# shamspias/fennec

Hardware: AMD Instinct MI355X
Metric: megapixels/sec: 4K SSIMFast+GaussianBlur (higher is better)
Workload: dtype u8 (blur: exact int32 sums of 24-bit fixed-point weights on the i8 matrix pipe; fp64 SSIM)

## Files before the change

### fennec_amd/csrc/blur_mfma.hip

```cpp
#include <hip/hip_ext.h>

#include "blur_launch.hpp"
#include "devutil.hpp"

#include <algorithm>
#include <cmath>
#include <type_traits>
#include <vector>

namespace fnx {

typedef int v4i __attribute__((ext_vector_type(4)));

constexpr int MF_P = 48;
constexpr int MF_WT = 64 * MF_P + 256;
constexpr int MF_SP = 352;
constexpr int MF_OP = 272;

__host__ __device__ constexpr int mf_skew(int grp) { return 80 * grp; }
static_assert(64 * MF_P + mf_skew(3) <= MF_WT, "the ring's last group ends inside the wave's ring");

struct MfmaArgs {
    const uint8_t *src;
    const uint8_t *const *srcs;
    uint8_t *dst;
    uint8_t *const *dsts;
    int sstride, dstride, w, h;
    int tiles_x, tiles, seg;
    int radius;
    const uint32_t *tab;
    int seed_h, seed_v, thr;
    const int32_t *bx, *by;
    const uint32_t *coltab, *rowtab;
    unsigned long long *slabs;
    int nbx, nby;
    int dbg;
    int narrow;
};

__device__ __forceinline__ int mf_comb3(int hi, int mid, int lo)
{
    int t = hi * 256 + mid;
    asm volatile("" : "+v"(t));
    return t * 256 + lo;
}

__device__ __forceinline__ const double *mf_scalar_ptr(const double *p)
{
    const unsigned long long v = reinterpret_cast<unsigned long long>(p);
    const unsigned lo = __builtin_amdgcn_readfirstlane(static_cast<unsigned>(v)), hi = __builtin_amdgcn_readfirstlane(static_cast<unsigned>(v >> 32));
    return reinterpret_cast<const double *>((static_cast<unsigned long long>(hi) << 32) | lo);
}
typedef __attribute__((address_space(1))) uint8_t mf_g_u8;
template <typename T> __device__ __forceinline__ T *mf_sgpr_ptr(T *p)
{
    unsigned long long v = reinterpret_cast<unsigned long long>(p);
    asm volatile("" : "+s"(v));
    return reinterpret_cast<T *>(v);
}
__device__ __forceinline__ void mf_lane_off(uint32_t &o) { asm volatile("" : "+v"(o)); }
typedef int mf_s16i __attribute__((ext_vector_type(16)));
__device__ __forceinline__ uint32_t mf_exact_u(const double *wd, const uint8_t *base, int step, int ring0, int mask)
{
    mf_s16i w0, w1;
    asm volatile("s_load_dwordx16 %0, %2, 0x0\n\ts_load_dwordx16 %1, %2, 0x40\n\ts_waitcnt lgkmcnt(0)" : "=&s"(w0), "=&s"(w1) : "s"(mf_scalar_ptr(wd)) : "memory");
    uint32_t v[13];
#pragma unroll
    for (int t = 0; t < 13; t++) v[t] = base[((ring0 + t) & mask) * step];
    double acc = 0;
#pragma unroll
    for (int t = 0; t < 13; t++) {
        const int lo = t < 8 ? w0[2 * (t & 7)] : w1[2 * (t & 7)], hi = t < 8 ? w0[2 * (t & 7) + 1] : w1[2 * (t & 7) + 1];
        acc = acc + u8_to_f64(v[t] ^ 0x80u) * __hiloint2double(hi, lo);
    }
    return clampF_dev(acc);
}

__device__ __forceinline__ void mf_box_add4(uint32_t *tbl, const u32x4 ro, uint32_t coln, const v4i cb, bool live)
{
    if (!live) return;
#pragma unroll
    for (int k = 0; k < 4; k++)
        __hip_atomic_fetch_add(reinterpret_cast<uint32_t *>(reinterpret_cast<char *>(tbl) + ro[k] + coln), static_cast<uint32_t>(cb[k]),
                               __ATOMIC_RELAXED, __HIP_MEMORY_SCOPE_WORKGROUP);
}

template <bool SCORE, bool GUARD>
__global__ __launch_bounds__(256, GUARD ? 3 : 1) void blur_mfma_kernel(MfmaArgs a)
{
    constexpr int P = MF_P, WT = MF_WT, SP = MF_SP, OP = MF_OP;
    __shared__ __attribute__((aligned(16))) uint8_t s_t[4 * WT];
    __shared__ __attribute__((aligned(16))) uint8_t s_stage[2 * 16 * SP];
    __shared__ __attribute__((aligned(16))) uint8_t s_out[2 * 16 * OP];
    __shared__ __attribute__((aligned(16))) uint32_t s_rowh[SCORE ? MF_SEG_SCORE + 32 : 4];
    __shared__ __attribute__((aligned(16))) uint32_t s_rowv[SCORE ? MF_SEG_SCORE + 16 : 4];
    extern __shared__ __attribute__((aligned(16))) uint32_t s_box[];

    const int tile = xcd_tile(blockIdx.x, a.tiles);
    if (tile < 0) return;
    const int z = blockIdx.y;
    const uint8_t *src = a.srcs ? a.srcs[z] : a.src;
    uint8_t *dst = a.dsts ? a.dsts[z] : a.dst;
    const int ty = tile / a.tiles_x, tx = tile - ty * a.tiles_x;
    const int x0 = tx * 64, y0 = ty * a.seg;
    const int tid = threadIdx.x, wave = tid >> 6, lane = tid & 63;
    const int r = lane & 15, g = lane >> 4;
    const int NJ = min(a.seg, ((a.h - y0 + 15) >> 4) << 4) >> 4;
    const int NI = NJ + 1;
    const bool xedge = x0 - 6 < 0 || x0 + 70 > a.w;

    const v4i *tbh = reinterpret_cast<const v4i *>(a.tab);
    const long *tbv = reinterpret_cast<const long *>(a.tab + 3 * 64 * 4);
    const v4i bh2 = tbh[lane], bh1 = tbh[64 + lane], bh0 = tbh[128 + lane];
    const long bv2 = tbv[lane], bv1 = tbv[64 + lane], bv0 = tbv[128 + lane];
    const bool alane = (r & 3) == 3;
    const int seed_hl = alane ? (1 << 23) + 128 : a.seed_h;
    const v4i sh = {seed_hl, seed_hl, seed_hl, seed_hl}, sv = {a.seed_v, a.seed_v, a.seed_v, a.seed_v};
    const v4i zero = {0, 0, 0, 0};
    const uint32_t sel01 = alane ? 0x0c0c0400u : 0x0c0c0703u, sel23 = alane ? 0x04000c0cu : 0x07030c0cu;

    uint8_t *tw = s_t + wave * WT;
    const int id1 = min(256 + tid, 16 * 19 - 1);
    const int srow0 = tid / 19, sch0 = tid - 19 * srow0, srow1 = id1 / 19, sch1 = id1 - 19 * srow1;
    const bool two = tid < 48;
    const int st_w0 = srow0 * SP + 16 * sch0, st_w1 = srow1 * SP + 16 * sch1;
    const int st_r = r * SP + 64 * wave + 16 * g;
    uint8_t *t_w = tw + r * P + 4 * g;
    const int m4 = r >> 2, mi = r & 3;
    const uint8_t *t_r = tw + (16 * m4 + 4 * mi) * P + mf_skew(m4) + 8 * g;
    const uint8_t *t_ro = tw + (16 * m4 + 4 * mi) * P + mf_skew(m4) + ((8 * g + 16) & 31);
    const uint8_t *t_ae = tw + (16 * g + 3) * P + mf_skew(g) + r + 6;
    const uint8_t *t_ao = tw + (16 * g + 3) * P + mf_skew(g) + ((r + 22) & 31);
    const int o_w = r * OP + 64 * wave + 16 * g;
    const int orow = tid >> 4, och = tid & 15;
    const int o_r = orow * OP + 16 * och;
    const int xo = x0 + 4 * och;

    v4i bbox = {0, 0, 0, 0}, sbox = {0, 0, 0, 0};
    uint32_t coln = 0;
    bool live = false;
    const int slabn = SCORE ? (a.nbx + 1) * (a.nby + 1) : 0;
    uint32_t *tbl_s = s_box, *tbl_b = s_box + 4 * slabn;
    auto score_setup = [&]() {
        const uint32_t cw = a.coltab[256 * tx + tid];
        const int nrow = (2 * a.seg + 16) >> 2;
        const int nrh = (a.seg + 16) >> 2;
        const u32x4 rw = reinterpret_cast<const u32x4 *>(a.rowtab)[static_cast<size_t>(ty) * nrow + min(tid, nrow - 1)];
        if (!(a.dbg & 4)) for (int e = tid; e < 2 * slabn; e += 256) reinterpret_cast<u32x4 *>(s_box)[e] = (u32x4){0u, 0u, 0u, 0u};
        if (tid < nrh) reinterpret_cast<u32x4 *>(s_rowh)[tid] = rw;
        else if (tid < nrow) reinterpret_cast<u32x4 *>(s_rowv)[tid - nrh] = rw;
        coln = cw & 0xfffffu;
        live = cw >> 31;
        const int seed = static_cast<int>((cw >> 20) & 31u) << 7;
        sbox = (v4i){seed, seed, seed, seed};
        const uint32_t sh = ((cw >> 29) & 3u) << 3;
#pragma unroll
        for (int e = 0; e < 4; e++) bbox[e] = static_cast<int>(((cw >> (25 + e)) & 1u) << sh);
    };

    const double *wd = reinterpret_cast<const double *>(a.tab + 3 * 64 * 4 + 3 * 64 * 2);

    auto stage_write = [&](const u32x4 (&d)[2], int buf) {
        uint8_t *sb = s_stage + buf * 16 * SP;
        *reinterpret_cast<u32x4 *>(sb + st_w0) = d[0] ^ 0x80808080u;
        if (two) *reinterpret_cast<u32x4 *>(sb + st_w1) = d[1] ^ 0x80808080u;
    };
    auto hset = [&](int s, int buf, int slot) {
        const uint8_t *sbuf = s_stage + buf * 16 * SP;
        const uint8_t *sb = sbuf + st_r;
        if constexpr (!GUARD && !SCORE) {
#pragma unroll
            for (int hf = 0; hf < 2; hf++) {
                v4i c2[2], c1[2], c0[2];
#pragma unroll
                for (int q2 = 0; q2 < 2; q2++) {
                    const v4i A = *reinterpret_cast<const v4i *>(sb + 16 * (2 * hf + q2));
                    c2[q2] = __builtin_amdgcn_mfma_i32_16x16x64_i8(A, bh2, zero, 0, 0, 0);
                    c1[q2] = __builtin_amdgcn_mfma_i32_16x16x64_i8(A, bh1, zero, 0, 0, 0);
                    c0[q2] = __builtin_amdgcn_mfma_i32_16x16x64_i8(A, bh0, sh, 0, 0, 0);
                }
#pragma unroll
// ... 125 lines not shown
            if (__builtin_amdgcn_ballot_w64(mm < static_cast<uint32_t>(a.thr))) {
                uint32_t fl = 0;
#pragma unroll
                for (int q = 0; q < 3; q++)
#pragma unroll
                    for (int i = 0; i < 4; i++) fl |= ((static_cast<uint32_t>(u[q][i]) & 0x00ffffffu) < static_cast<uint32_t>(a.thr) ? 1u : 0u) << (4 * q + i);
                unsigned long long todo = __builtin_amdgcn_ballot_w64(fl != 0);
                while (todo) {
                    const int L = __builtin_ctzll(todo);
                    todo &= todo - 1;
                    uint32_t flL = __builtin_amdgcn_readlane(fl, L);
                    const int rL = L & 15, gL = L >> 4;
                    while (flL) {
                        const int b = __builtin_ctz(flL), q = b >> 2, i = b & 3;
                        flL &= flL - 1;
                        const uint32_t e = mf_exact_u(wd, tw + (16 * gL + 4 * i + q) * P + mf_skew(gL), 1, (ODD ? 16 : 0) + rL, 31);
                        if (lane == L) op[4 * i + q] = static_cast<uint8_t>(e);
                    }
                }
                if constexpr (SCORE) o = *reinterpret_cast<const u32x4 *>(op);
            }
        }
        if constexpr (SCORE) {
            const u32x4 os = o ^ 0x80808080u;
            const v4i A = {(int)os[0], (int)os[1], (int)os[2], (int)os[3]};
            const v4i cb = __builtin_amdgcn_mfma_i32_16x16x64_i8(A, bbox, sbox, 0, 0, 0);
            const u32x4 ro = *reinterpret_cast<const u32x4 *>(s_rowv + 16 * j + 4 * g);
            if (!(a.dbg & 1)) mf_box_add4(tbl_b, ro, coln, cb, live);
        }
    };

    auto march = [&](auto formt) {
        constexpr int FORM = decltype(formt)::value;
        constexpr bool XEDGE = FORM == 2, INNER = FORM == 0;
        const uint8_t *in_base = INNER ? src + static_cast<ptrdiff_t>(y0 - 6) * a.sstride + 4 * static_cast<ptrdiff_t>(x0 - 6) : src;
        uint8_t *out_base = INNER ? dst + static_cast<ptrdiff_t>(y0) * a.dstride + 4 * static_cast<ptrdiff_t>(x0) : dst;
        const uint32_t ss = static_cast<uint32_t>(a.sstride), ds = static_cast<uint32_t>(a.dstride);
        const uint32_t in_set = 16u * ss, out_set = 16u * ds;
        uint32_t in_l0 = static_cast<uint32_t>(srow0) * ss + 16u * sch0, in_l1 = static_cast<uint32_t>(srow1) * ss + 16u * sch1;
        uint32_t out_l = static_cast<uint32_t>(orow) * ds + 16u * och;
        auto hload = [&](int i, u32x4 (&d)[2]) {
            const int ys = y0 - 6 + 16 * i;
            if constexpr (INNER) {
                const mf_g_u8 *sb = (const mf_g_u8 *)mf_sgpr_ptr(in_base + static_cast<uint32_t>(i) * in_set);
                mf_lane_off(in_l0);
                mf_lane_off(in_l1);
                d[0] = *(g_u32x4 *)(sb + in_l0);
                d[1] = *(g_u32x4 *)(sb + in_l1);
            } else if constexpr (!XEDGE) {
                const uint8_t *sb = src + 4 * static_cast<ptrdiff_t>(x0 - 6);
                const int ya = clampi(ys + srow0, 0, a.h - 1), yb = clampi(ys + srow1, 0, a.h - 1);
                d[0] = *(g_u32x4 *)(sb + static_cast<ptrdiff_t>(ya) * a.sstride + 16 * sch0);
                d[1] = *(g_u32x4 *)(sb + static_cast<ptrdiff_t>(yb) * a.sstride + 16 * sch1);
            } else {
    #pragma unroll
                for (int k = 0; k < 2; k++) {
                    if (k == 1 && !two) break;
                    const int y = clampi(ys + (k ? srow1 : srow0), 0, a.h - 1);
                    const uint8_t *rowp = src + static_cast<size_t>(y) * a.sstride;
                    const int xc = x0 - 6 + 4 * (k ? sch1 : sch0);
    #pragma unroll
                    for (int e = 0; e < 4; e++) d[k][e] = ld_px(rowp, clampi(xc + e, 0, a.w - 1));
                }
            }
        };
        auto out_store = [&](int j, int buf) {
            const u32x4 o = *reinterpret_cast<const u32x4 *>(s_out + buf * 16 * OP + o_r);
            if constexpr (INNER) {
                mf_lane_off(out_l);
                *(g_u32x4w *)((mf_g_u8 *)mf_sgpr_ptr(out_base + static_cast<uint32_t>(j) * out_set) + out_l) = o;
                return;
            }
            const int y = y0 + 16 * j + orow;
            if (y < a.h) {
                uint8_t *dp = dst + static_cast<size_t>(y) * a.dstride + 4 * static_cast<size_t>(xo);
                if (!XEDGE || xo + 3 < a.w) *(g_u32x4w *)(dp) = o;
                else {
    #pragma unroll
                    for (int e = 0; e < 4; e++) if (xo + e < a.w) *(g_u32w *)(dp + 4 * e) = o[e];
                }
            }
        };
        u32x4 ra[2], rb[2];
        hload(0, ra);
        __builtin_amdgcn_sched_barrier(0);
        hload(min(1, NI - 1), rb);
        __builtin_amdgcn_sched_barrier(0);
        if constexpr (SCORE) score_setup();
        auto step = [&](int s, u32x4 (&d)[2], auto oddv) {
            constexpr int par = decltype(oddv)::value ? 0 : 1;
            if (s < NI) stage_write(d, par);
            if (XEDGE) { if (s + 2 < NI) hload(s + 2, d); } else hload(min(s + 2, NI - 1), d);
            if (s >= 3 && s - 3 < NJ) out_store(s - 3, par);
            __syncthreads();
            if (s < NI) hset(s, par, par);
            if (s >= 1 && s - 1 < NJ) vset(s - 1, par, oddv);
        };
    #pragma unroll 1
        for (int s = 0; s < NJ + 3; s += 2) {
            step(s, ra, std::true_type{});
            step(s + 1, rb, std::false_type{});
        }

    };
    const bool inner = !xedge && a.narrow && y0 >= 6 && y0 + 16 * NJ + 10 <= a.h;
    if (xedge) march(std::integral_constant<int, 2>{});
    else if (inner) march(std::integral_constant<int, 0>{});
    else march(std::integral_constant<int, 1>{});

    if (SCORE && !(a.dbg & 2)) {
        __syncthreads();
        unsigned long long *slab = a.slabs + (static_cast<size_t>(z) * a.tiles + tile) * 2 * slabn;
        for (int e = tid; e < 2 * slabn; e += 256) {
            const u32x4 v = *reinterpret_cast<const u32x4 *>(s_box + 4 * e);
            slab[e] = static_cast<unsigned long long>(v.x | (v.y << 16)) | (static_cast<unsigned long long>(v.z) << 32);
        }
    }
}

template <int NKH> struct MfWide {
    static constexpr int NKV = mf_wide_nkv(NKH);
    static constexpr int RF = mf_wide_rf(NKH);
    static constexpr int NC = 16 + RF / 2;
    static constexpr int NL = (16 * NC + 255) / 256;
    static constexpr int SP = 16 * NC + 48;
    static constexpr int NT = 2 * RF + 1;
    static constexpr int NS = 4 * NKV;
    static constexpr int RING = 16 * NS;
    static constexpr int P = RING + 16;
    static constexpr int WT = 64 * P + 256;
};

template <int NT>
__device__ __noinline__ uint32_t mf_exact_h_n(const uint8_t *p, const double *wd)
{
    double acc = 0;
#pragma unroll 15
    for (int t = 0; t < NT; t++) acc = acc + u8_to_f64(p[4 * t] ^ 0x80u) * wd[t];
    return clampF_dev(acc);
}
template <int NT, int RING = 64>
__device__ __noinline__ uint32_t mf_exact_v_n(const uint8_t *p, int ring0, const double *wd)
{
    double acc = 0;
#pragma unroll 15
    for (int t = 0; t < NT; t++) acc = acc + u8_to_f64(p[static_cast<unsigned>(ring0 + t) % static_cast<unsigned>(RING)] ^ 0x80u) * wd[t];
    return clampF_dev(acc);
}
// ... 368 lines not shown
    case 2: return mfma_wide_kernel<2>(p.exact, score);
    case 3: return mfma_wide_kernel<3>(p.exact, score);
    case 4: return mfma_wide_kernel<4>(p.exact, score);
    case 5: return mfma_wide_kernel<5>(p.exact, score);
    case 6: return mfma_wide_kernel<6>(p.exact, score);
    case 7: return mfma_wide_kernel<7>(p.exact, score);
    case 8: return mfma_wide_kernel<8>(p.exact, score);
    }
    return nullptr;
}

int launch_blur_mfma(fnx_ctx *ctx, int n, const BlurPlan &p, const BlurImages &im, const double *kernel, const BlurScore *score)
{
    const bool wide = p.family == BLUR_MFMA_WIDE;
    const MfmaKernel kern = mfma_kernel(p, score != nullptr);
    if (!kern) return FNX_ERR_INVALID;
    MfmaArgs ma{};
    set_images(ma, im);
    const std::vector<uint32_t> tab = mfma_table(p, kernel);
    void *dt = nullptr;
    FNX_TRY(upload_table(ctx, SLOT_TABLE_MFMA, tab.data(), sizeof(uint32_t) * tab.size(), &dt));
    ma.tab = static_cast<const uint32_t *>(dt);
    ma.radius = p.radius;
    ma.seed_h = p.seed_h; ma.seed_v = p.seed_v; ma.thr = p.thr;
    ma.seg = score ? score->seg : p.seg;
    ma.tiles_x = (ma.w + 63) / 64;
    ma.tiles = ma.tiles_x * ((ma.h + ma.seg - 1) / ma.seg);
    const dim3 grid(8 * ((ma.tiles + 7) / 8), n);
    size_t lds = 0;
    if (score) {
        if (wide) { ma.bx = score->bx; ma.by = score->by; }
        else { ma.coltab = score->coltab; ma.rowtab = score->rowtab; }
        ma.slabs = score->slabs; ma.nbx = score->nbx; ma.nby = score->nby;
        lds = sizeof(uint32_t) * 8 * static_cast<size_t>(ma.nbx + 1) * (ma.nby + 1);
    }
    if (!wide) {
#ifdef FNX_DEVELOP
        { static const int dbg = [] { const char *e = dev_env("FNX_MFMA_DBG"); return e ? atoi(e) : 0; }(); ma.dbg = dbg; }
#endif
        auto fits = [&](int stride) {
            return stride > 0 && stride < (1 << 24) &&
                   static_cast<long long>(ma.h - 1) * stride + 4LL * ma.w + 16LL * stride < (1LL << 31);
        };
        ma.narrow = fits(ma.sstride) && fits(ma.dstride);
    }
    LaunchEvents ev;
    FNX_TRY(blur_bind_events(ctx, score != nullptr, &ev));
    note_route(ctx, FNX_PROF_MAIN, blur_route(p, score != nullptr));
    hipExtLaunchKernelGGL(kern, grid, dim3(256), lds, ctx->stream, ev.start, ev.stop, 0, ma);
    FNX_HIP(hipGetLastError());
    return FNX_OK;
}

}

extern "C" int fnx_blur_fixed_point(const double *kernel, int radius, long long *wq, double *err255)
{
    if (!kernel || !wq || !err255) {
        fnx::set_error("invalid argument: fnx_blur_fixed_point");
        return FNX_ERR_INVALID;
    }
    fnx::MfmaWeights q;
    if (!fnx::mfma_quantise(kernel, radius, &q, fnx::MF_RWIDE)) return FNX_NOOP;
    for (int i = 0; i < 2 * radius + 1; i++) wq[i] = q.wq[i];
    *err255 = q.err255;
    return FNX_OK;
}
```

### fennec_amd/csrc/common.hpp

```cpp
#pragma once
#include <hip/hip_runtime.h>

#include <cstdarg>
#include <cstdint>
#include <cstdio>
#include <cstdlib>
#include <cstring>
#include <vector>

#include "../../include/fennec_hip.h"
#include "blur_plan.hpp"
#include "dev_env.hpp"
#include "png_compress_plan.hpp"

namespace fnx {

void set_error(const char *fmt, ...);


enum Form {
    FORM_FX_STREAM = 0,
    FORM_FX_PAIRS,
    FORM_FX_REF,
    FORM_RESIZE_MFMA,
    FORM_RESIZE_FP64,
    FORM_RESIZE_FUSED,
    FORM_MSSSIM_LEVELWISE,
    FORM_MSSSIM_NOFUSE0,
    FORM_MSSSIM_FOLD,
    FORM_MSSSIM_BOXFLY,
    FORM_PALETTE_GRID,
    FORM_RESIZE_BOX,
    FORM_JPEG_SIZE,
    FORM_COUNT
};

#define FNX_HIP(expr)                                                                      \
    do {                                                                                   \
        hipError_t e__ = (expr);                                                           \
        if (e__ != hipSuccess) {                                                           \
            fnx::set_error("%s failed: %s (%s:%d)", #expr, hipGetErrorString(e__), __FILE__, \
                           __LINE__);                                                      \
            return e__ == hipErrorOutOfMemory ? FNX_ERR_OOM : FNX_ERR_HIP;                 \
        }                                                                                  \
    } while (0)

#define FNX_TRY(expr)            \
    do {                         \
        int r__ = (expr);        \
        if (r__ < 0) return r__; \
    } while (0)

#define FNX_REQUIRE(cond, msg)                  \
    do {                                        \
        if (!(cond)) {                          \
            fnx::set_error("invalid argument: %s", msg); \
            return FNX_ERR_INVALID;             \
        }                                       \
    } while (0)

enum Slot {
    SLOT_IN_A = 0,
    SLOT_IN_B,
    SLOT_OUT,
    SLOT_TMP0,
// ... 586 lines not shown
```

### fennec_amd/csrc/runtime.cpp

```cpp
#include "common.hpp"

#include <dlfcn.h>

#include <atomic>
#include <cstdlib>
#include <cstring>
#include <mutex>
#include <string>
#include <vector>

namespace fnx {

namespace {
std::mutex g_dev_mu;
bool g_dev_set = false;
std::vector<int> g_devmap;

int hip_device_count()
{
    int n = 0;
    if (hipGetDeviceCount(&n) != hipSuccess) {
        (void)hipGetLastError();
        return 0;
    }
// ... 35 lines not shown
    int st = g_roctx_state.load(std::memory_order_acquire);
    if (st == 0) {
        std::lock_guard<std::mutex> lk(g_dev_mu);
        st = g_roctx_state.load(std::memory_order_relaxed);
        if (st == 0) {
            st = 2;
            const char *e = std::getenv("FNX_ROCTX");
            if (e && e[0] == '1') {
                for (const char *lib : {"librocprofiler-sdk-roctx.so", "librocprofiler-sdk-roctx.so.1", "libroctx64.so", "libroctx64.so.4"}) {
                    void *h = dlopen(lib, RTLD_NOW | RTLD_GLOBAL);
                    if (!h) continue;
                    g_roctx_push = reinterpret_cast<roctx_push_fn>(dlsym(h, "roctxRangePushA"));
                    g_roctx_pop = reinterpret_cast<roctx_pop_fn>(dlsym(h, "roctxRangePop"));
                    if (g_roctx_push && g_roctx_pop) { st = 1; break; }
                }
            }
            g_roctx_state.store(st, std::memory_order_release);
        }
    }
    return st == 1;
}
}

OpRange::OpRange(const char *name) : on_(roctx_on())
{
    if (on_) g_roctx_push(name);
}
OpRange::~OpRange()
{
    if (on_) g_roctx_pop();
}

static const char *const FORM_NAMES[FORM_COUNT] = {"fx_stream", "fx_pairs", "fx_ref", "resize_mfma", "resize_fp64", "resize_fused",
                                                   "msssim_levelwise", "msssim_nofuse0", "msssim_fold", "msssim_boxfly", "palette_grid", "resize_box", "jpeg_size"};

const char *form_value(const fnx_ctx *ctx, Form f)
{
    if (ctx && ctx->form[f][0]) return ctx->form[f];
#ifdef FNX_DEVELOP
    char name[40] = "FNX_";
    size_t k = 4;
    for (const char *p = FORM_NAMES[f]; *p && k + 1 < sizeof(name); p++) name[k++] = static_cast<char>(*p >= 'a' && *p <= 'z' ? *p - 32 : *p);
    name[k] = 0;
    return std::getenv(name);
#else
    return nullptr;
#endif
}

int form_set(fnx_ctx *ctx, const char *name, const char *value)
{
    for (int f = 0; f < FORM_COUNT; f++) {
        if (std::strcmp(name, FORM_NAMES[f]) != 0) continue;
        if (value && std::strlen(value) >= sizeof(ctx->form[f])) { set_error("fnx_ctx_set_form: value too long"); return FNX_ERR_INVALID; }
        std::memset(ctx->form[f], 0, sizeof(ctx->form[f]));
        if (value) std::strcpy(ctx->form[f], value);
        return FNX_OK;
    }
    set_error("fnx_ctx_set_form: no kernel form called '%s'", name);
    return FNX_ERR_INVALID;
}

static thread_local char g_err[512] = "";

void set_error(const char *fmt, ...)
{
    va_list ap;
// ... 521 lines not shown
```

### fennec_amd/csrc/blur_plan.cpp

```cpp
#include "blur_plan.hpp"

#include <algorithm>
#include <cmath>
#include <cstdlib>
#include <cstring>

#include "box_edge.hpp"
#include "dev_env.hpp"

namespace fnx {

bool mfma_quantise(const double *kernel, int radius, MfmaWeights *q, int rmax)
{
    if (radius < 1 || radius > rmax) return false;
    const int nt = 2 * radius + 1;
    double sum = 0;
    for (int i = 0; i < nt; i++) {
        if (!(kernel[i] >= 0) || !(kernel[i] < 0.49)) return false;
        sum += kernel[i];
    }
    if (!(std::fabs(sum - 1.0) <= 1e-6)) return false;
    long long tot = 0;
    for (int i = 0; i < nt; i++) {
        q->wq[i] = std::llround(kernel[i] * 16777216.0);
// ... 99 lines not shown
}

static void score_mfma_tables(ScoreGeom &g, int w, int h)
{
    const int seg = g.th, nbx = g.nbx, nby = g.nby;
    const int tiles_x = (w + 63) / 64, segs = (h + seg - 1) / seg;
    const size_t ref_words = 4 * (static_cast<size_t>(g.dstW) + g.dstH);
    const size_t base = (NHEAD + ref_words + static_cast<size_t>(w) + h + 3) & ~size_t(3);
    g.coltab = base;
    g.rowtab = base + 256 * static_cast<size_t>(tiles_x);
    g.map.resize(g.rowtab + static_cast<size_t>(segs) * (2 * seg + 16), 0);
    const int32_t *bx = g.map.data() + NHEAD + ref_words, *by = bx + w;
    uint32_t *col = reinterpret_cast<uint32_t *>(g.map.data()) + g.coltab, *row = reinterpret_cast<uint32_t *>(g.map.data()) + g.rowtab;
    for (int tx = 0; tx < tiles_x; tx++) {
        const int x0 = 64 * tx;
        uint32_t colbox[64];
        const int b0x = bx[x0];
        for (int i = 0; i < 64; i++) {
            const int v = x0 + i < w ? bx[x0 + i] : -1;
            colbox[i] = (v >= 0 && b0x >= 0) ? static_cast<uint32_t>(v - b0x) : 255u;
        }
        for (int wave = 0; wave < 4; wave++) {
            uint32_t first = 255u;
            for (int i = 0; i < 16; i++) first = std::min(first, colbox[16 * wave + i]);
            for (int lane = 0; lane < 64; lane++) {
                const int r = lane & 15, gq = lane >> 4;
                const int slot = r / 3, ch = r - 3 * slot;
                uint32_t cnt = 0, in = 0;
                for (int i = 0; i < 16; i++) cnt += (r < 15 && colbox[16 * wave + i] == first + slot) ? 1 : 0;
                for (int e = 0; e < 4; e++)
                    if (r < 15 && first != 255u && colbox[16 * wave + 4 * gq + e] == first + slot) in |= 1u << e;
                const bool live = r < 15 && first != 255u && cnt > 0;
                const uint32_t bc = live ? first + slot : static_cast<uint32_t>(nbx);
                const uint32_t coln = 16u * bc + 4u * (r < 15 ? ch : 3);
                col[(4 * tx + wave) * 64 + lane] = coln | cnt << 20 | in << 25 | static_cast<uint32_t>(ch) << 29 | (live ? 1u << 31 : 0u);
            }
        }
    }
    const int rowbytes = 16 * (nbx + 1);
    for (int ty = 0; ty < segs; ty++) {
        const int y0 = ty * seg, b0y = by[y0];
        uint32_t *rh = row + static_cast<size_t>(ty) * (2 * seg + 16), *rv = rh + seg + 16;
        auto off = [&](int t) {
            const int v = (t >= 0 && t < seg && y0 + t < h) ? by[y0 + t] : -1;
            return static_cast<uint32_t>(rowbytes * ((v >= 0 && b0y >= 0) ? v - b0y : nby));
        };
        for (int u = 0; u < seg + 16; u++) rh[u] = off(u - 6);
        for (int t = 0; t < seg; t++) rv[t] = off(t);
    }
}
static bool build_score_geom(ScoreGeom &g, int w, int h, int radius, int dstW, int dstH, int th_fixed = 0)
{
    if (radius < 1 || radius > (th_fixed ? mf_wide_rf(MF_SCORE_NKH) : SCORE_RMAX) || w < dstW || h < dstH || dstW <= 0 || dstH <= 0 || w >= (1 << 24) ||
        h >= (1 << 24))
        return false;
    const double xr = static_cast<double>(w) / static_cast<double>(dstW);
    const double yr = static_cast<double>(h) / static_cast<double>(dstH);
    if (std::fmin(xr, yr) < 3.6) return false;
    const size_t ref_words = 4 * (static_cast<size_t>(dstW) + dstH);
    std::vector<int32_t> &map = g.map;
    map.assign(NHEAD + ref_words + static_cast<size_t>(w) + h, -1);
    {
        uint32_t *magic = reinterpret_cast<uint32_t *>(map.data()), *tiedown = magic + 260;
        std::fill(magic, magic + NHEAD, 0u);
        for (uint32_t c = 1; c <= 256; c++) {
            magic[c] = static_cast<uint32_t>((1ull << 32) / (2ull * c)) + 1u;
            if (c & 1u) continue;
            const double inv = 1.0 / static_cast<double>(c);
            for (uint32_t k = 0; k < 256; k++) {
                const double n = static_cast<double>(c / 2) * static_cast<double>(2 * k + 1);
                if (n > 255.0 * c) break;
                if (n * inv < static_cast<double>(k) + 0.5) tiedown[8 * c + (k >> 5)] |= 1u << (k & 31);
            }
        }
    }
    BoxRef *xref = reinterpret_cast<BoxRef *>(map.data() + NHEAD), *yref = xref + dstW;
    int32_t *bx = map.data() + NHEAD + ref_words, *by = bx + w;
    int maxbw = 0, maxbh = 0;
    for (int d = 0; d < dstW; d++) {
        int s0, s1;
        box_edge(d, xr, w, s0, s1);
        if (d + 1 < dstW) { int n0, n1; box_edge(d + 1, xr, w, n0, n1); if (n0 < s1) return false; }
        for (int x = s0; x < s1; x++) bx[x] = d;
        if (s1 - s0 > maxbw) maxbw = s1 - s0;
    }
    for (int d = 0; d < dstH; d++) {
        int s0, s1;
        box_edge(d, yr, h, s0, s1);
        if (d + 1 < dstH) { int n0, n1; box_edge(d + 1, yr, h, n0, n1); if (n0 < s1) return false; }
        for (int y = s0; y < s1; y++) by[y] = d;
        if (s1 - s0 > maxbh) maxbh = s1 - s0;
    }
    if (static_cast<long>(maxbw) * maxbh > 256) return false;
    bool tall = g.tall_pref;
    int th = 0, nbx = 0, nby = 0;
    for (int attempt = 0; attempt < (th_fixed ? 1 : 2); attempt++, tall = !tall) {
        th = th_fixed ? th_fixed : direct_tile_rows(radius, tall);
        nbx = nby = 1;
        auto span = [](const int32_t *m, int lo, int hi) {
            int first = -1, last = -1;
            for (int i = lo; i < hi; i++)
                if (m[i] >= 0) { if (first < 0) first = m[i]; last = m[i]; }
            return first < 0 ? 0 : last - first + 1;
        };
        for (int x0 = 0; x0 < w; x0 += 64) nbx = std::max(nbx, span(bx, x0, std::min(w, x0 + 64)));
        for (int y0 = 0; y0 < h; y0 += th) nby = std::max(nby, span(by, y0, std::min(h, y0 + th)));
        if ((nbx + 1) * (nby + 1) <= (th_fixed > 272 ? 2 * SCORE_NBOX : SCORE_NBOX)) break;
        th = 0;
    }
    if (!th) return false;
    tall = th == direct_tile_rows(radius, true);
    if (th_fixed) {
        for (int x0 = 0; x0 < w; x0 += 16) {
            int first = -1, last = -1;
            for (int x = x0; x < std::min(w, x0 + 16); x++)
                if (bx[x] >= 0) { if (first < 0) first = bx[x]; last = bx[x]; }
            if (first >= 0 && last - first > 4) return false;
        }
    }
    for (int x0 = 0; x0 < w; x0 += 64)
        if (bx[x0] < 0) for (int x = x0; x < std::min(w, x0 + 64); x++) if (bx[x] >= 0) return false;
    for (int y0 = 0; y0 < h; y0 += th)
        if (by[y0] < 0) for (int y = y0; y < std::min(h, y0 + th); y++) if (by[y] >= 0) return false;

    const int slabn = (nbx + 1) * (nby + 1);
    const int tiles_x = (w + 63) / 64, tiles = tiles_x * ((h + th - 1) / th);
    if (static_cast<size_t>(tiles) * 2 * slabn >= (1u << 30)) return false;
    for (int d = 0; d < dstW; d++) {
        int s0, s1;
        box_edge(d, xr, w, s0, s1);
        const int t0 = s0 >> 6, t1 = (s1 - 1) >> 6;
        if (t1 > t0 + 1) return false;
        xref[d].part0 = t0 * 2 * slabn + (d - bx[t0 << 6]);
        xref[d].part1 = t1 > t0 ? t1 * 2 * slabn + (d - bx[t1 << 6]) : -1;
        xref[d].len = s1 - s0; xref[d].pad = 0;
    }
    for (int d = 0; d < dstH; d++) {
        int s0, s1;
        box_edge(d, yr, h, s0, s1);
        const int t0 = s0 / th, t1 = (s1 - 1) / th;
        if (t1 > t0 + 1) return false;
        yref[d].part0 = t0 * tiles_x * 2 * slabn + (d - by[t0 * th]) * (nbx + 1);
        yref[d].part1 = t1 > t0 ? t1 * tiles_x * 2 * slabn + (d - by[t1 * th]) * (nbx + 1) : -1;
        yref[d].len = s1 - s0; yref[d].pad = 0;
    }

    g.th = th; g.nbx = nbx; g.nby = nby; g.tall = tall;
    g.coltab = g.rowtab = 0;
    if (th_fixed && th_fixed <= 272 && radius <= 6) score_mfma_tables(g, w, h);
    return true;
}

static bool plan_matrix(BlurPlan &p, int num_cus, int n, int w, int h, const double *kernel)
{
    static const bool off = [] { const char *e = dev_env("FNX_BLUR_MFMA"); return e && e[0] == '0'; }();
    static const bool exact_on = [] { const char *e = dev_env("FNX_BLUR_MFMA_EXACT"); return !(e && e[0] == '0'); }();
    static const int cap = [] { const char *e = dev_env("FNX_MFMA_SEG"); return e ? atoi(e) : MF_SEG; }();
    if (off || (p.exact && !exact_on) || n > 65535 || w < 64 || h < 32 || !mfma_quantise(kernel, p.radius, &p.q, MF_RWIDE)) return false;
    p.gq = p.exact ? static_cast<long long>(std::ceil(p.q.err255)) + 2 : 0;
    if (p.gq > (1 << 20)) return false;
    p.seed_h = static_cast<int>((1u << 23) + static_cast<uint32_t>(p.gq));
    p.seed_v = static_cast<int>((1u << 23) + (1u << 31) + static_cast<uint32_t>(p.gq));
    p.thr = static_cast<int>(2 * p.gq);
    if (p.radius <= MF_RMAX) {
        p.family = BLUR_MFMA;
        p.seg = blur_mfma_segment(num_cus, n, w, h, cap, p.exact ? 3 : 4);
    } else {
        p.family = BLUR_MFMA_WIDE;
        for (p.nkh = 2; p.radius > mf_wide_rf(p.nkh); p.nkh++) {}
        p.seg = blur_mfma_segment(num_cus, n, w, h, MF_SEG, 3);
    }
    return true;
}

BlurPlan plan_blur(int num_cus, int n, int w, int h, const double *kernel, int radius, bool exact)
{
    BlurPlan p;
    p.num_cus = num_cus; p.n = n; p.w = w; p.h = h; p.radius = radius;
    p.exact = exact;
    if (plan_matrix(p, num_cus, n, w, h, kernel)) return p;
    if (radius < 1 || radius > FUSED_RMAX) {
        p.family = exact || radius > 26 ? BLUR_GENERIC_F64 : BLUR_GENERIC_F32;
    } else if (!exact || guard_kernel_ok(kernel, radius)) {
        p.family = BLUR_DIRECT;
        p.tall = direct_tall(num_cus, radius, n, w, h);
        p.wdp = exact && radius > SCORE_RMAX;
    } else {
        p.family = radius > SCORE_RMAX ? BLUR_GENERIC_F64 : BLUR_EXACT;
    }
    return p;
}

const char *blur_route(const BlurPlan &p, bool score)
{
    static const char *const names[3][4] = {
        {"blur_mfma_kernel", "blur_mfma_kernel<GUARD>", "blur_mfma_kernel<SCORE>", "blur_mfma_kernel<SCORE, GUARD>"},
        {"blur_mfma_wide_kernel", "blur_mfma_wide_kernel<GUARD>", "blur_mfma_wide_kernel<SCORE>", "blur_mfma_wide_kernel<SCORE, GUARD>"},
        {"blur_direct_kernel", "blur_direct_kernel<GUARD>", "blur_direct_kernel<SCORE>", "blur_direct_kernel<SCORE, GUARD>"}};
    if (p.family <= BLUR_DIRECT) return names[p.family][(score ? 2 : 0) + (p.exact ? 1 : 0)];
    return p.family == BLUR_EXACT ? "blur_exact_kernel" : (p.family == BLUR_GENERIC_F64 ? "blur_pass_kernel<double> x 2" : "blur_pass_kernel<float> x 2");
}

bool plan_blur_scored(const BlurPlan &p, int dstW, int dstH, ScoreGeom &g)
{
    const int num_cus = p.num_cus, n = p.n, w = p.w, h = p.h;
    static const int wide_cap = [] { const char *e = dev_env("FNX_MFMA_WIDE_SEG"); return e ? atoi(e) : MF_SEG_SCORE_WIDE; }();
    if (n > 65535) return false;
    int seg = 0;
    bool tall_pref = false;
    switch (p.family) {
    case BLUR_MFMA: seg = blur_mfma_segment(num_cus, n, w, h, MF_SEG_SCORE, 3); break;
    case BLUR_MFMA_WIDE:
        if (p.nkh > MF_SCORE_NKH) return false;
        seg = blur_mfma_segment(num_cus, n, w, h, wide_cap, 2);
        break;
    case BLUR_DIRECT:
        if (p.radius > SCORE_RMAX) return false;
        tall_pref = p.tall;
        break;
    default: return false;
    }
    const int radius = p.radius;
    if (!(g.w == w && g.h == h && g.dstW == dstW && g.dstH == dstH && g.radius == radius && g.tall_pref == tall_pref && g.seg == seg)) {
        g.w = w; g.h = h; g.dstW = dstW; g.dstH = dstH; g.radius = radius; g.tall_pref = tall_pref; g.seg = seg;
        g.mfma = seg > 0 && build_score_geom(g, w, h, radius, dstW, dstH, seg);
        g.ok = seg > 0 ? g.mfma : build_score_geom(g, w, h, radius, dstW, dstH);
    }
    return g.ok && g.th <= (p.family == BLUR_MFMA ? MF_SEG_SCORE : MF_SEG_SCORE_WIDE);
}

}
```

### fennec_amd/csrc/blur_plan.hpp

```cpp
#pragma once
#include <cstddef>
#include <cstdint>
#include <vector>

namespace fnx {

constexpr int MF_RMAX = 6;
constexpr int MF_RWIDE = 62;
constexpr int MF_SEG_SCORE = 272;
constexpr int MF_SEG_SCORE_WIDE = 544;
constexpr int MF_SEG = 544;
constexpr int mf_wide_nkv(int nkh) { return nkh <= 4 ? 1 : (nkh <= 7 ? 2 : 3); }
constexpr int mf_wide_rf(int nkh) { return 8 * nkh - 2 < 32 * mf_wide_nkv(nkh) - 8 ? 8 * nkh - 2 : 32 * mf_wide_nkv(nkh) - 8; }
constexpr int MF_SCORE_NKH = 4;
constexpr int FUSED_RMAX = 16;
constexpr int SCORE_RMAX = 8;
constexpr int WIDE_IH = 128;
constexpr int SCORE_NBOX = 512;
constexpr int NHEAD = 260 + 257 * 8;
struct BoxRef {
    int32_t part0, part1;
    int32_t len, pad;
};

struct MfmaWeights {
    long long wq[2 * MF_RWIDE + 1];
    double err255;
};
bool mfma_quantise(const double *kernel, int radius, MfmaWeights *q, int rmax = MF_RMAX);
constexpr size_t MF_TAB_WORDS = 3 * 64 * 4 + 3 * 64 * 2;
constexpr size_t MF_TAB_ALL = MF_TAB_WORDS + 2 * 16;
constexpr size_t mf_wide_tab_words(int nkh) { return (3 * nkh + 3 * mf_wide_nkv(nkh)) * 64 * 4; }
constexpr size_t mf_wide_tab_all(int nkh) { return mf_wide_tab_words(nkh) + 2 * ((2 * mf_wide_rf(nkh) + 1 + 7) / 8 * 8); }

enum BlurFamily {
    BLUR_MFMA = 0,
    BLUR_MFMA_WIDE,
    BLUR_DIRECT,
    BLUR_EXACT,
    BLUR_GENERIC_F32,
    BLUR_GENERIC_F64
};
struct BlurPlan {
    BlurFamily family = BLUR_GENERIC_F64;
    int num_cus = 0, n = 0, w = 0, h = 0, radius = 0;
    bool exact = false;
    int nkh = 0;
    bool tall = false;
    bool wdp = false;
    int seg = 0;
    MfmaWeights q = {};
    long long gq = 0;
    int seed_h = 0, seed_v = 0, thr = 0;
};

struct ScoreGeom {
    int w = 0, h = 0, dstW = 0, dstH = 0, radius = 0;
    bool tall_pref = false, tall = false, ok = false;
    bool mfma = false;
    int seg = 0;
    int th = 0, nbx = 0, nby = 0;
    std::vector<int32_t> map;
    size_t coltab = 0, rowtab = 0;
};

BlurPlan plan_blur(int num_cus, int n, int w, int h, const double *kernel, int radius, bool exact);
bool plan_blur_scored(const BlurPlan &p, int dstW, int dstH, ScoreGeom &g);
const char *blur_route(const BlurPlan &p, bool score);
std::vector<uint32_t> mfma_table(const BlurPlan &p, const double *kernel);

}
```

Baseline: 456,400.

## Add scalar-base edge-row march form for top/bottom blur tiles

Adds a fourth march form for tiles touching the top or bottom image edge in narrow-stride cases. Interior steps use the scalar-base, 32-bit-offset loads and stores of the inner path. Only the final steps switch to a clamped-row loader and a masked store. Previously these tiles took the generic clamped path for every row. A form option can restore the old clamped behaviour. The cost is more template instantiations and code size.

```diff
diff --git a/fennec_amd/csrc/blur_mfma.hip b/fennec_amd/csrc/blur_mfma.hip
--- a/fennec_amd/csrc/blur_mfma.hip
+++ b/fennec_amd/csrc/blur_mfma.hip
@@ -5,6 +5,7 @@
 
 #include <algorithm>
 #include <cmath>
+#include <cstring>
 #include <type_traits>
 #include <vector>
 
@@ -36,6 +37,7 @@
     int nbx, nby;
     int dbg;
     int narrow;
+    int clamp_rows;
 };
 
 __device__ __forceinline__ int mf_comb3(int hi, int mid, int lo)
@@ -338,17 +340,18 @@
 
     auto march = [&](auto formt) {
         constexpr int FORM = decltype(formt)::value;
-        constexpr bool XEDGE = FORM == 2, INNER = FORM == 0;
-        const uint8_t *in_base = INNER ? src + static_cast<ptrdiff_t>(y0 - 6) * a.sstride + 4 * static_cast<ptrdiff_t>(x0 - 6) : src;
-        uint8_t *out_base = INNER ? dst + static_cast<ptrdiff_t>(y0) * a.dstride + 4 * static_cast<ptrdiff_t>(x0) : dst;
+        constexpr bool XEDGE = FORM == 2, INNER = FORM == 0, EDGEY = FORM == 3, SBASE = INNER || EDGEY;
+        constexpr int RB = EDGEY ? 10 : 0, IB = EDGEY ? 1 : 0;
+        const uint8_t *in_base = SBASE ? src + static_cast<ptrdiff_t>(EDGEY ? y0 : y0 - 6) * a.sstride + 4 * static_cast<ptrdiff_t>(x0 - 6) : src;
+        uint8_t *out_base = SBASE ? dst + static_cast<ptrdiff_t>(y0) * a.dstride + 4 * static_cast<ptrdiff_t>(x0) : dst;
         const uint32_t ss = static_cast<uint32_t>(a.sstride), ds = static_cast<uint32_t>(a.dstride);
         const uint32_t in_set = 16u * ss, out_set = 16u * ds;
-        uint32_t in_l0 = static_cast<uint32_t>(srow0) * ss + 16u * sch0, in_l1 = static_cast<uint32_t>(srow1) * ss + 16u * sch1;
+        uint32_t in_l0 = static_cast<uint32_t>(srow0 + RB) * ss + 16u * sch0, in_l1 = static_cast<uint32_t>(srow1 + RB) * ss + 16u * sch1;
         uint32_t out_l = static_cast<uint32_t>(orow) * ds + 16u * och;
         auto hload = [&](int i, u32x4 (&d)[2]) {
             const int ys = y0 - 6 + 16 * i;
-            if constexpr (INNER) {
-                const mf_g_u8 *sb = (const mf_g_u8 *)mf_sgpr_ptr(in_base + static_cast<uint32_t>(i) * in_set);
+            if constexpr (SBASE) {
+                const mf_g_u8 *sb = (const mf_g_u8 *)mf_sgpr_ptr(in_base + static_cast<uint32_t>(i - IB) * in_set);
                 mf_lane_off(in_l0);
                 mf_lane_off(in_l1);
                 d[0] = *(g_u32x4 *)(sb + in_l0);
@@ -370,11 +373,21 @@
                 }
             }
         };
-        auto out_store = [&](int j, int buf) {
+        int er0 = srow0, ec0 = 16 * sch0, er1 = srow1, ec1 = 16 * sch1, eor = orow;
+        auto hload_edge = [&](int i, u32x4 (&d)[2]) {
+            const int ys = y0 - 6 + 16 * i, yb = clampi(ys, 0, a.h - 1);
+            const mf_g_u8 *sb = (const mf_g_u8 *)mf_sgpr_ptr(src + static_cast<ptrdiff_t>(yb) * a.sstride + 4 * static_cast<ptrdiff_t>(x0 - 6));
+            const uint32_t l0 = static_cast<uint32_t>(clampi(ys + er0, 0, a.h - 1) - yb) * ss + static_cast<uint32_t>(ec0);
+            const uint32_t l1 = static_cast<uint32_t>(clampi(ys + er1, 0, a.h - 1) - yb) * ss + static_cast<uint32_t>(ec1);
+            d[0] = *(g_u32x4 *)(sb + l0);
+            d[1] = *(g_u32x4 *)(sb + l1);
+        };
+        auto out_store = [&](int j, int buf, auto lastt) {
             const u32x4 o = *reinterpret_cast<const u32x4 *>(s_out + buf * 16 * OP + o_r);
-            if constexpr (INNER) {
+            if constexpr (SBASE) {
                 mf_lane_off(out_l);
-                *(g_u32x4w *)((mf_g_u8 *)mf_sgpr_ptr(out_base + static_cast<uint32_t>(j) * out_set) + out_l) = o;
+                if (!decltype(lastt)::value || eor < a.h - y0 - 16 * j)
+                    *(g_u32x4w *)((mf_g_u8 *)mf_sgpr_ptr(out_base + static_cast<uint32_t>(j) * out_set) + out_l) = o;
                 return;
             }
             const int y = y0 + 16 * j + orow;
@@ -388,30 +401,44 @@
             }
         };
         u32x4 ra[2], rb[2];
-        hload(0, ra);
+        if constexpr (EDGEY) hload_edge(0, ra); else hload(0, ra);
         __builtin_amdgcn_sched_barrier(0);
-        hload(min(1, NI - 1), rb);
+        if constexpr (EDGEY) hload_edge(1, rb); else hload(min(1, NI - 1), rb);
         __builtin_amdgcn_sched_barrier(0);
         if constexpr (SCORE) score_setup();
-        auto step = [&](int s, u32x4 (&d)[2], auto oddv) {
+        auto step = [&](int s, u32x4 (&d)[2], auto oddv, auto lastt) {
             constexpr int par = decltype(oddv)::value ? 0 : 1;
             if (s < NI) stage_write(d, par);
-            if (XEDGE) { if (s + 2 < NI) hload(s + 2, d); } else hload(min(s + 2, NI - 1), d);
-            if (s >= 3 && s - 3 < NJ) out_store(s - 3, par);
+            if constexpr (decltype(lastt)::value) hload_edge(min(s + 2, NI - 1), d);
+            else if (XEDGE) { if (s + 2 < NI) hload(s + 2, d); } else hload(min(s + 2, NI - 1), d);
+            if (s >= 3 && s - 3 < NJ) out_store(s - 3, par, lastt);
             __syncthreads();
             if (s < NI) hset(s, par, par);
             if (s >= 1 && s - 1 < NJ) vset(s - 1, par, oddv);
         };
+        const int sb = EDGEY && y0 + 16 * NJ + 10 > a.h ? max(0, (NI - 4) & ~1) : NJ + 3;
     #pragma unroll 1
-        for (int s = 0; s < NJ + 3; s += 2) {
-            step(s, ra, std::true_type{});
-            step(s + 1, rb, std::false_type{});
-        }
-
+        for (int s = 0; s < sb; s += 2) {
+            step(s, ra, std::true_type{}, std::false_type{});
+            step(s + 1, rb, std::false_type{}, std::false_type{});
+        }
+        if constexpr (EDGEY) {
+            int t = tid;
+            asm volatile("" : "+v"(t));
+            const int i1 = min(256 + t, 16 * 19 - 1);
+            er0 = t / 19; ec0 = 16 * (t - 19 * er0); er1 = i1 / 19; ec1 = 16 * (i1 - 19 * er1); eor = t >> 4;
+    #pragma unroll 1
+            for (int s = sb; s < NJ + 3; s += 2) {
+                step(s, ra, std::true_type{}, std::true_type{});
+                step(s + 1, rb, std::false_type{}, std::true_type{});
+            }
+        }
     };
-    const bool inner = !xedge && a.narrow && y0 >= 6 && y0 + 16 * NJ + 10 <= a.h;
-    if (xedge) march(std::integral_constant<int, 2>{});
-    else if (inner) march(std::integral_constant<int, 0>{});
+    const bool inner = y0 >= 6 && y0 + 16 * NJ + 10 <= a.h;
+    const int form = xedge ? 2 : (!a.narrow || (a.dbg & 8)) ? 1 : inner ? 0 : a.clamp_rows ? 1 : 3;
+    if (form == 2) march(std::integral_constant<int, 2>{});
+    else if (form == 0) march(std::integral_constant<int, 0>{});
+    else if (form == 3) march(std::integral_constant<int, 3>{});
     else march(std::integral_constant<int, 1>{});
 
     if (SCORE && !(a.dbg & 2)) {
@@ -865,6 +892,8 @@
                    static_cast<long long>(ma.h - 1) * stride + 4LL * ma.w + 16LL * stride < (1LL << 31);
         };
         ma.narrow = fits(ma.sstride) && fits(ma.dstride);
+        const char *rows = form_value(ctx, FORM_BLUR_ROWS);
+        ma.clamp_rows = rows && std::strcmp(rows, "clamp") == 0;
     }
     LaunchEvents ev;
     FNX_TRY(blur_bind_events(ctx, score != nullptr, &ev));
diff --git a/fennec_amd/csrc/common.hpp b/fennec_amd/csrc/common.hpp
--- a/fennec_amd/csrc/common.hpp
+++ b/fennec_amd/csrc/common.hpp
@@ -31,6 +31,7 @@
     FORM_MSSSIM_BOXFLY,
     FORM_PALETTE_GRID,
     FORM_RESIZE_BOX,
+    FORM_BLUR_ROWS,
     FORM_JPEG_SIZE,
     FORM_COUNT
 };
diff --git a/fennec_amd/csrc/runtime.cpp b/fennec_amd/csrc/runtime.cpp
--- a/fennec_amd/csrc/runtime.cpp
+++ b/fennec_amd/csrc/runtime.cpp
@@ -91,7 +91,8 @@
 }
 
 static const char *const FORM_NAMES[FORM_COUNT] = {"fx_stream", "fx_pairs", "fx_ref", "resize_mfma", "resize_fp64", "resize_fused",
-                                                   "msssim_levelwise", "msssim_nofuse0", "msssim_fold", "msssim_boxfly", "palette_grid", "resize_box", "jpeg_size"};
+                                                   "msssim_levelwise", "msssim_nofuse0", "msssim_fold", "msssim_boxfly", "palette_grid", "resize_box", "blur_rows",
+                                                   "jpeg_size"};
 
 const char *form_value(const fnx_ctx *ctx, Form f)
 {
```

Result: no change. 458,700 (median of 6 runs) (+0.5%).

## Pack score box accumulators to 12 bytes and size segment cap from LDS budget

Applied to the files above, without the earlier changes.

Shrinks each per-box atomic accumulator entry in LDS from 16 to 12 bytes and derives the maximum box count from an explicit LDS budget. The scored MFMA path's segment height is now capped by a host-side computation that finds the tallest segment whose box table fits. The intent is to keep the scored blur on the fast MFMA path with the largest segment that fits LDS, and to reduce LDS footprint so occupancy can hold. This risks misaligned three-word reads in the slab flush and adds host-side planning work, though that work is cached.

```diff
diff --git a/fennec_amd/csrc/blur_mfma.hip b/fennec_amd/csrc/blur_mfma.hip
--- a/fennec_amd/csrc/blur_mfma.hip
+++ b/fennec_amd/csrc/blur_mfma.hip
@@ -92,9 +92,12 @@
     __shared__ __attribute__((aligned(16))) uint8_t s_t[4 * WT];
     __shared__ __attribute__((aligned(16))) uint8_t s_stage[2 * 16 * SP];
     __shared__ __attribute__((aligned(16))) uint8_t s_out[2 * 16 * OP];
-    __shared__ __attribute__((aligned(16))) uint32_t s_rowh[SCORE ? MF_SEG_SCORE + 32 : 4];
-    __shared__ __attribute__((aligned(16))) uint32_t s_rowv[SCORE ? MF_SEG_SCORE + 16 : 4];
+    __shared__ __attribute__((aligned(16))) uint32_t s_rowh[SCORE ? MF_SEG_SCORE_MAX + 32 : 4];
+    __shared__ __attribute__((aligned(16))) uint32_t s_rowv[SCORE ? MF_SEG_SCORE_MAX + 16 : 4];
     extern __shared__ __attribute__((aligned(16))) uint32_t s_box[];
+    static_assert(sizeof(s_t) + sizeof(s_stage) + sizeof(s_out) == MF_LDS_FIXED, "blur_plan.hpp's LDS budget counts these arrays");
+    static_assert(!SCORE || MF_LDS_FIXED + sizeof(s_rowh) + sizeof(s_rowv) == MF_LDS_SCORE_STATIC, "... and the row tables");
+    static_assert((2 * MF_SEG_SCORE_MAX + 16) / 4 <= 256, "score_setup: one 16-byte chunk of the row tables per thread");
 
     const int tile = xcd_tile(blockIdx.x, a.tiles);
     if (tile < 0) return;
@@ -140,13 +143,13 @@
     uint32_t coln = 0;
     bool live = false;
     const int slabn = SCORE ? (a.nbx + 1) * (a.nby + 1) : 0;
-    uint32_t *tbl_s = s_box, *tbl_b = s_box + 4 * slabn;
+    uint32_t *tbl_s = s_box, *tbl_b = s_box + 3 * slabn;
     auto score_setup = [&]() {
         const uint32_t cw = a.coltab[256 * tx + tid];
         const int nrow = (2 * a.seg + 16) >> 2;
         const int nrh = (a.seg + 16) >> 2;
         const u32x4 rw = reinterpret_cast<const u32x4 *>(a.rowtab)[static_cast<size_t>(ty) * nrow + min(tid, nrow - 1)];
-        if (!(a.dbg & 4)) for (int e = tid; e < 2 * slabn; e += 256) reinterpret_cast<u32x4 *>(s_box)[e] = (u32x4){0u, 0u, 0u, 0u};
+        if (!(a.dbg & 4)) for (int e = tid; e < (6 * slabn + 3) >> 2; e += 256) reinterpret_cast<u32x4 *>(s_box)[e] = (u32x4){0u, 0u, 0u, 0u};
         if (tid < nrh) reinterpret_cast<u32x4 *>(s_rowh)[tid] = rw;
         else if (tid < nrow) reinterpret_cast<u32x4 *>(s_rowv)[tid - nrh] = rw;
         coln = cw & 0xfffffu;
@@ -418,8 +421,8 @@
         __syncthreads();
         unsigned long long *slab = a.slabs + (static_cast<size_t>(z) * a.tiles + tile) * 2 * slabn;
         for (int e = tid; e < 2 * slabn; e += 256) {
-            const u32x4 v = *reinterpret_cast<const u32x4 *>(s_box + 4 * e);
-            slab[e] = static_cast<unsigned long long>(v.x | (v.y << 16)) | (static_cast<unsigned long long>(v.z) << 32);
+            const uint32_t *v = s_box + 3 * e;
+            slab[e] = static_cast<unsigned long long>(v[0] | (v[1] << 16)) | (static_cast<unsigned long long>(v[2]) << 32);
         }
     }
 }
@@ -854,7 +857,8 @@
         if (wide) { ma.bx = score->bx; ma.by = score->by; }
         else { ma.coltab = score->coltab; ma.rowtab = score->rowtab; }
         ma.slabs = score->slabs; ma.nbx = score->nbx; ma.nby = score->nby;
-        lds = sizeof(uint32_t) * 8 * static_cast<size_t>(ma.nbx + 1) * (ma.nby + 1);
+        const size_t entries = static_cast<size_t>(ma.nbx + 1) * (ma.nby + 1);
+        lds = wide ? sizeof(uint32_t) * 8 * entries : (2 * MF_BOX_ENTRY * entries + 15) & ~size_t(15);
     }
     if (!wide) {
 #ifdef FNX_DEVELOP
diff --git a/fennec_amd/csrc/blur_plan.cpp b/fennec_amd/csrc/blur_plan.cpp
--- a/fennec_amd/csrc/blur_plan.cpp
+++ b/fennec_amd/csrc/blur_plan.cpp
@@ -155,12 +155,12 @@
                     if (r < 15 && first != 255u && colbox[16 * wave + 4 * gq + e] == first + slot) in |= 1u << e;
                 const bool live = r < 15 && first != 255u && cnt > 0;
                 const uint32_t bc = live ? first + slot : static_cast<uint32_t>(nbx);
-                const uint32_t coln = 16u * bc + 4u * (r < 15 ? ch : 3);
+                const uint32_t coln = MF_BOX_ENTRY * bc + 4u * (r < 15 ? ch : 0);
                 col[(4 * tx + wave) * 64 + lane] = coln | cnt << 20 | in << 25 | static_cast<uint32_t>(ch) << 29 | (live ? 1u << 31 : 0u);
             }
         }
     }
-    const int rowbytes = 16 * (nbx + 1);
+    const int rowbytes = MF_BOX_ENTRY * (nbx + 1);
     for (int ty = 0; ty < segs; ty++) {
         const int y0 = ty * seg, b0y = by[y0];
         uint32_t *rh = row + static_cast<size_t>(ty) * (2 * seg + 16), *rv = rh + seg + 16;
@@ -215,6 +215,9 @@
         if (s1 - s0 > maxbh) maxbh = s1 - s0;
     }
     if (static_cast<long>(maxbw) * maxbh > 256) return false;
+    const bool narrow = th_fixed && radius <= MF_RMAX;
+    if (narrow && (th_fixed > MF_SEG_SCORE_MAX || th_fixed % 16)) return false;
+    const int nbox = narrow ? MF_SCORE_NBOX : (th_fixed > 272 ? 2 * SCORE_NBOX : SCORE_NBOX);
     bool tall = g.tall_pref;
     int th = 0, nbx = 0, nby = 0;
     for (int attempt = 0; attempt < (th_fixed ? 1 : 2); attempt++, tall = !tall) {
@@ -228,7 +231,7 @@
         };
         for (int x0 = 0; x0 < w; x0 += 64) nbx = std::max(nbx, span(bx, x0, std::min(w, x0 + 64)));
         for (int y0 = 0; y0 < h; y0 += th) nby = std::max(nby, span(by, y0, std::min(h, y0 + th)));
-        if ((nbx + 1) * (nby + 1) <= (th_fixed > 272 ? 2 * SCORE_NBOX : SCORE_NBOX)) break;
+        if ((nbx + 1) * (nby + 1) <= nbox) break;
         th = 0;
     }
     if (!th) return false;
@@ -270,7 +273,7 @@
 
     g.th = th; g.nbx = nbx; g.nby = nby; g.tall = tall;
     g.coltab = g.rowtab = 0;
-    if (th_fixed && th_fixed <= 272 && radius <= 6) score_mfma_tables(g, w, h);
+    if (narrow) score_mfma_tables(g, w, h);
     return true;
 }
 
@@ -324,15 +327,59 @@
     return p.family == BLUR_EXACT ? "blur_exact_kernel" : (p.family == BLUR_GENERIC_F64 ? "blur_pass_kernel<double> x 2" : "blur_pass_kernel<float> x 2");
 }
 
+static int score_seg_cap(int w, int h, int dstW, int dstH)
+{
+    if (dstW <= 0 || dstH <= 0 || w < dstW || h < dstH) return 16;
+    const double xr = static_cast<double>(w) / static_cast<double>(dstW), yr = static_cast<double>(h) / static_cast<double>(dstH);
+    std::vector<int32_t> lo(static_cast<size_t>(std::max(w, h)), -1), hi;
+    for (int d = 0; d < dstW; d++) {
+        int s0, s1;
+        box_edge(d, xr, w, s0, s1);
+        for (int x = s0; x < s1; x++) lo[x] = d;
+    }
+    int nbx = 1;
+    for (int x0 = 0; x0 < w; x0 += 64) {
+        int first = -1, last = -1;
+        for (int x = x0; x < std::min(w, x0 + 64); x++)
+            if (lo[x] >= 0) { if (first < 0) first = lo[x]; last = lo[x]; }
+        if (first >= 0) nbx = std::max(nbx, last - first + 1);
+    }
+    std::fill(lo.begin(), lo.end(), -1);
+    for (int d = 0; d < dstH; d++) {
+        int s0, s1;
+        box_edge(d, yr, h, s0, s1);
+        for (int y = s0; y < s1; y++) lo[y] = d;
+    }
+    hi.assign(lo.begin(), lo.begin() + h);
+    for (int y = 1; y < h; y++) if (hi[y] < 0) hi[y] = hi[y - 1];
+    for (int y = h - 2; y >= 0; y--) if (lo[y] < 0) lo[y] = lo[y + 1];
+    for (int seg = MF_SEG_SCORE_MAX; seg > 16; seg -= 16) {
+        int nby = 1;
+        for (int y0 = 0; y0 < h; y0++) {
+            const int first = lo[y0], last = hi[std::min(h, y0 + seg) - 1];
+            if (first >= 0 && last >= first) nby = std::max(nby, last - first + 1);
+        }
+        if ((nbx + 1) * (nby + 1) <= MF_SCORE_NBOX) return seg;
+    }
+    return 16;
+}
+
 bool plan_blur_scored(const BlurPlan &p, int dstW, int dstH, ScoreGeom &g)
 {
     const int num_cus = p.num_cus, n = p.n, w = p.w, h = p.h;
     static const int wide_cap = [] { const char *e = dev_env("FNX_MFMA_WIDE_SEG"); return e ? atoi(e) : MF_SEG_SCORE_WIDE; }();
+    static const int score_cap = [] { const char *e = dev_env("FNX_MFMA_SCORE_SEG"); return e && *e ? std::max(16, atoi(e) & ~15) : MF_SEG_SCORE_MAX; }();
     if (n > 65535) return false;
     int seg = 0;
     bool tall_pref = false;
     switch (p.family) {
-    case BLUR_MFMA: seg = blur_mfma_segment(num_cus, n, w, h, MF_SEG_SCORE, 3); break;
+    case BLUR_MFMA:
+        if (!(g.cap > 0 && g.cap_w == w && g.cap_h == h && g.cap_dstW == dstW && g.cap_dstH == dstH)) {
+            g.cap_w = w; g.cap_h = h; g.cap_dstW = dstW; g.cap_dstH = dstH;
+            g.cap = std::min(score_cap, score_seg_cap(w, h, dstW, dstH));
+        }
+        seg = blur_mfma_segment(num_cus, n, w, h, g.cap, 3);
+        break;
     case BLUR_MFMA_WIDE:
         if (p.nkh > MF_SCORE_NKH) return false;
         seg = blur_mfma_segment(num_cus, n, w, h, wide_cap, 2);
@@ -349,7 +396,7 @@
         g.mfma = seg > 0 && build_score_geom(g, w, h, radius, dstW, dstH, seg);
         g.ok = seg > 0 ? g.mfma : build_score_geom(g, w, h, radius, dstW, dstH);
     }
-    return g.ok && g.th <= (p.family == BLUR_MFMA ? MF_SEG_SCORE : MF_SEG_SCORE_WIDE);
-}
-
-}
+    return g.ok && g.th <= (p.family == BLUR_MFMA ? MF_SEG_SCORE_MAX : MF_SEG_SCORE_WIDE);
+}
+
+}
diff --git a/fennec_amd/csrc/blur_plan.hpp b/fennec_amd/csrc/blur_plan.hpp
--- a/fennec_amd/csrc/blur_plan.hpp
+++ b/fennec_amd/csrc/blur_plan.hpp
@@ -7,7 +7,12 @@
 
 constexpr int MF_RMAX = 6;
 constexpr int MF_RWIDE = 62;
-constexpr int MF_SEG_SCORE = 272;
+constexpr int MF_SEG_SCORE_MAX = 272;
+constexpr int MF_LDS_WORKGROUP = 53760;
+constexpr int MF_LDS_FIXED = 33280;
+constexpr int MF_LDS_SCORE_STATIC = MF_LDS_FIXED + 4 * ((MF_SEG_SCORE_MAX + 32) + (MF_SEG_SCORE_MAX + 16));
+constexpr int MF_BOX_ENTRY = 12;
+constexpr int MF_SCORE_NBOX = (MF_LDS_WORKGROUP - MF_LDS_SCORE_STATIC) / (2 * MF_BOX_ENTRY);
 constexpr int MF_SEG_SCORE_WIDE = 544;
 constexpr int MF_SEG = 544;
 constexpr int mf_wide_nkv(int nkh) { return nkh <= 4 ? 1 : (nkh <= 7 ? 2 : 3); }
@@ -59,6 +64,7 @@
     bool tall_pref = false, tall = false, ok = false;
     bool mfma = false;
     int seg = 0;
+    int cap = 0, cap_w = 0, cap_h = 0, cap_dstW = 0, cap_dstH = 0;
     int th = 0, nbx = 0, nby = 0;
     std::vector<int32_t> map;
     size_t coltab = 0, rowtab = 0;
```

Measured after the change: 441,800 before, 441,200 after. About the same (-0.1%).
